# mills-lab/vapor

Measured on AMD Instinct MI355X. Metric: SV loci validated/sec, higher is better.
Workload: dtype u32

## Files before the change

### vapor_amd/build.py

```python
from __future__ import annotations

import hashlib
import os
import re
import subprocess
import sys

HERE = os.path.dirname(os.path.abspath(__file__))
ROOT = os.path.dirname(HERE)
SO = os.path.join(HERE, "libvapor_hip.so")
CSRC = os.path.join(HERE, "csrc")
SOURCES = [os.path.join(CSRC, "vapor_hip.hip"), os.path.join(CSRC, "vapor_bam.cpp")]
_HEADERS = [("vapor_kernels.h", True), ("vapor_wide.h", True), ("vapor_anyk.h", True), ("vapor_inflate.h", False),
            ("vapor_bamdev.h", True), ("vapor_fasta.h", True), ("vapor_refine.h", True), ("vapor_bgzf.h", False),
            ("vapor_records.h", True), ("vapor_planner.h", False), ("vapor_names.h", True),
            ("vapor_readrec.h", True), ("vapor_readplan.h", False), ("vapor_sa.h", False),
            ("vapor_realign.h", True), ("vapor_realign_plan.h", True),
            ("vapor_band_row.h", True),
            ("vapor_realign_trace.h", True), ("vapor_trace_plan.h", True),
            ("vapor_polish.h", True), ("vapor_polish_plan.h", True),
            ("vapor_junction.h", True), ("vapor_junction_plan.h", True),
            ("vapor_revote.h", True), ("vapor_revote_plan.h", True),
            ("vapor_polish_call.h", False),
            ("vapor_seqset_plan.h", False), ("vapor_image.h", False)]
DEPS = SOURCES + [os.path.join(CSRC, h) for h, _dev in _HEADERS] + [os.path.join(ROOT, "include", "vapor_hip.h")]
KERNEL_FILES = [os.path.join(CSRC, h) for h, dev in _HEADERS if dev] + [SOURCES[0], os.path.abspath(__file__)]

EXTRA_FLAGS = ["-mllvm", "-amdgpu-atomic-optimizer-strategy=None", "-mllvm", "-amdgpu-sched-strategy=max-ilp"]


def hipcc() -> str:
    for c in (os.environ.get("HIPCC"), "/opt/rocm/bin/hipcc", "hipcc"):
        if c and (os.path.isabs(c) and os.path.exists(c) or not os.path.isabs(c)):
            return c
    raise RuntimeError("hipcc not found")


_ID_RE = re.compile(rb"VAPOR_SOURCE_ID=([0-9a-f]{16}:[0-9a-f]{16})")

# ... 42 lines not shown
```

### vapor_amd/csrc/vapor_hip.hip

```cpp
#include "vapor_kernels.h"
#include "vapor_wide.h"
#include "vapor_anyk.h"
#include "vapor_realign.h"
#include "vapor_realign_trace.h"
#include "vapor_polish.h"
#include "vapor_revote.h"
#include "vapor_polish_call.h"
#include "vapor_seqset_plan.h"
#include "vapor_junction.h"
#include "vapor_bamdev.h"
#include "vapor_bgzf.h"
#include "vapor_fasta.h"
#include "vapor_refine.h"
#include "vapor_planner.h"
#include "vapor_readplan.h"
#include "vapor_hip.h"

#include <unistd.h>

#include <algorithm>
#include <cstdio>
#include <cstdlib>
#include <cstring>
#include <new>
#include <numeric>
#include <map>
#include <memory>
#include <mutex>
#include <set>
#include <string>
// ... 47 lines not shown
    bool user_stream = false;
    uint8_t* h_stage = nullptr;
    uint8_t* d_stage = nullptr;
    size_t stage_cap = 0;
    std::vector<double> h_gt;
    double* d_gt = nullptr;
    int reads_per_task = MAX_READS_PER_TASK;
    int n_cus = 256;
    int join_tasks = 256;
    int join_align = 1;
    int64_t max_pair_cap = (int64_t)1 << 28;
    bool shared_join = true;
    int remap_in_clean = 1;
    int clean_order = 1;
    int clean_fit = 1;
    int64_t trace_budget = vapor_trace::BUDGET_DEFAULT;
    int64_t anyk_edit_pairs = ANYK_EDIT_PAIRS;
    int stage_threads = 3;
    bool attrs_set = false;
    uint32_t* d_crc_pow = nullptr;
    std::map<const uint8_t*, size_t> arenas;
    hipStream_t bam_stream = nullptr;
    int bam_stream_share = 0;
    int bam_cu_share = 0;
    hipEvent_t bam_ev[2] = {nullptr, nullptr};
    double bam_stats[7] = {0, 0, 0, 0, 0, 0, 0};
    hipEvent_t fasta_ev[2] = {nullptr, nullptr};
    double fasta_stats[6] = {0, 0, 0, 0, 0, 0};
    BlockPool pool;
};
// ... 98 lines not shown
    vapor_ctx* ctx = nullptr;
    int device = 0;
    int32_t n = 0;
    int32_t n_lit = 0;
    std::vector<SeqDesc> h;
    SeqDesc* d_seqs = nullptr;
    uint32_t *d_p2 = nullptr, *d_e1 = nullptr, *d_x4 = nullptr;
    size_t plane_chunks = 0;
    std::vector<std::vector<HSeg>> derived;
    std::vector<ShareGroup> groups;
    std::vector<int32_t> group_of, slot_of;
    uint8_t* d_raw = nullptr;
    std::vector<int64_t> raw_off;
};

struct vapor_plan : PlanLayout {
    vapor_ctx* ctx = nullptr;
    int device = 0;
    vapor_seqset* set = nullptr;
    int64_t n_pairs = 0;
    std::vector<int64_t> last_stats;
    int hcap_want = 4096;
    bool hcap_measured = false;
    int64_t total_cap = 0;
    DPair* d_pairs = nullptr;
    DTask* d_tasks = nullptr;
    DTask* d_atasks = nullptr;
    int join_align = 0;
    PlanParams params{};
    bool aligned_made = false;
    int last_table = 0;
    int32_t* d_task_pairs = nullptr;
    unsigned long long* d_hits = nullptr;
    uint8_t* d_hflags = nullptr;
    unsigned long long* d_nhits = nullptr;
    long long* d_stats = nullptr;
    long long* h_stats = nullptr;
    hipEvent_t ev[4] = {nullptr, nullptr, nullptr, nullptr};
    hipEvent_t ev_f[2] = {nullptr, nullptr};
    std::vector<std::array<hipEvent_t, 4>> ring;
    int ring_n = 0;
    bool overflow_final = false;
    double acc_ms[4] = {0, 0, 0, 0};
    int64_t acc_n = 0;
    double* h_loci = nullptr;
    hipEvent_t ev_t0 = nullptr;
    hipStream_t lane = nullptr;
    int lane_ix = -1;
    hipStream_t fin = nullptr;
    hipEvent_t ev_clean = nullptr;
    hipEvent_t ev_fin = nullptr;
    bool have_fin = false;
    hipEvent_t ev_last = nullptr;
    hipEvent_t ev_after = nullptr;
    bool have_last = false, have_after = false;
    double t_join = 0, t_clean = 0, t_total = 0;
    int n_retried = 0;
    bool ran = false;
    bool flags_valid = false;
    int64_t n_reads = 0, n_loci = 0;
    DRead* d_reads = nullptr;
    int32_t* d_locus_first = nullptr;
    double* d_gt = nullptr;
    bool own_gt = false;
    double* d_read_scores = nullptr;
    double* d_loci = nullptr;
    unsigned int* d_overflow = nullptr;
    int32_t* d_big_list = nullptr;
    unsigned int* h_overflow = nullptr;
// ... 136 lines not shown
    if (!strcmp(name, "shared_join")) {
        c->shared_join = v != 0;
        return VAPOR_OK;
    }
    if (!strcmp(name, "remap_in_clean")) {
        if (v < 0 || v > 2) return fail(VAPOR_E_ARG, "vapor_set_param: remap_in_clean is 0, 1 or 2");
        c->remap_in_clean = (int)v;
        return VAPOR_OK;
    }
    if (!strcmp(name, "clean_order")) {
        c->clean_order = v != 0 ? 1 : 0;
        return VAPOR_OK;
    }
    if (!strcmp(name, "clean_fit")) {
        c->clean_fit = v != 0;
        return VAPOR_OK;
    }
    if (!strcmp(name, "trace_budget")) {
        c->trace_budget = vapor_trace::budget_of(v);
        return VAPOR_OK;
    }
    if (!strcmp(name, "anyk_edit_pairs")) {
        if (v < 1) return fail(VAPOR_E_ARG, "anyk_edit_pairs out of range");
        c->anyk_edit_pairs = v;
        return VAPOR_OK;
    }
    if (!strcmp(name, "stage_threads")) {
        if (v < 1 || v > 64) return fail(VAPOR_E_ARG, "stage_threads out of range");
        c->stage_threads = (int)v;
        return VAPOR_OK;
// ... 689 lines not shown
    dfree(p->ctx, p->d_hflags); p->d_hflags = nullptr;
    dfree(p->ctx, p->d_nhits); p->d_nhits = nullptr;
    dfree(p->ctx, p->d_stats); p->d_stats = nullptr;
    plan_free_reads(p);
    dfree(p->ctx, p->d_shares); p->d_shares = nullptr;
    dfree(p->ctx, p->d_maps); p->d_maps = nullptr;
    dfree(p->ctx, p->d_serve); p->d_serve = nullptr;
    dfree(p->ctx, p->d_clean_order); p->d_clean_order = nullptr;
    plan_free_grid(p);
}

extern "C" int vapor_plan_destroy(vapor_plan* p)
{
    if (!p) return VAPOR_OK;
    (void)hipSetDevice(p->device);
    if (p->ring_n > 0 && p->lane && ctx_alive(p->ctx)) {
        (void)hipStreamSynchronize(p->lane);
        if (p->fin) (void)hipStreamSynchronize(p->fin);
    }
    if (ctx_alive(p->ctx))
        for (auto& q : p->ctx->lane_plan)
            if (q == p) q = nullptr;
    plan_free_device(p);
    hfree(p->ctx, p->h_stats);
    hfree(p->ctx, p->h_overflow);
    dfree(p->ctx, p->d_overflow);
    dfree(p->ctx, p->d_big_list);
    for (auto& e : p->ev)
        if (e) (void)hipEventDestroy(e);
    for (auto& r : p->ring)
        for (auto& e : r)
            if (e) (void)hipEventDestroy(e);
    hfree(p->ctx, p->h_loci);
    for (auto& e : p->ev_f)
        if (e) (void)hipEventDestroy(e);
    if (p->ev_t0) (void)hipEventDestroy(p->ev_t0);
    if (p->ev_last) (void)hipEventDestroy(p->ev_last);
    if (p->ev_clean) (void)hipEventDestroy(p->ev_clean);
    if (p->ev_fin) (void)hipEventDestroy(p->ev_fin);
    if (p->ev_after) (void)hipEventDestroy(p->ev_after);
    delete p;
    return VAPOR_OK;
}

static_assert((2 * VAPOR_MAX_SEQ_LEN + 2 + 31) / 32 <= CLEAN_RANGE_WORDS_MAX, "cluster_axis sizes its per-thread word list for this");

static int plan_alloc_hits(vapor_plan* p)
{
    int64_t tot = 0;
    for (auto& d : p->hp) {
        d.hit_off = tot;
        tot += (int64_t)((d.cap + 3u) & ~3u);
    }
    tot += 4;
    HIPCHK(hipStreamSynchronize(p->ctx->stream));
    dfree(p->ctx, p->d_hits); p->d_hits = nullptr;
    dfree(p->ctx, p->d_hflags); p->d_hflags = nullptr;
    HIPCHK(dmalloc(p->ctx, (void**)&p->d_hits, (size_t)tot * sizeof(unsigned long long)));
    HIPCHK(dmalloc(p->ctx, (void**)&p->d_hflags, (size_t)tot));
    p->total_cap = tot;
// ... 17 lines not shown
    std::unique_ptr<vapor_plan, Building<vapor_plan, vapor_plan_destroy>> p(new (std::nothrow) vapor_plan(), {&sc});
    if (!p) return fail(VAPOR_E_NOMEM, "out of memory");
    p->ctx = ctx;
    p->device = ctx->device;
    p->set = set;
    p->n_pairs = n_pairs;
    p->params = PlanParams{ctx->reads_per_task, ctx->join_tasks, ctx->max_pair_cap, ctx->shared_join,
                           tile_pos<JoinCfg, 2>(), tile_pos<JoinCfg, 4>(), ctx->join_align == 2};
    static_cast<PlanLayout&>(*p) = plan_layout(p->params,
                                               SetView{set->h, set->n, set->n_lit, set->derived, set->groups, set->group_of, set->slot_of},
                                               n_pairs, pairs);
    p->join_align = ctx->join_align;
    if (p->join_align == 2) { p->tasks = p->atasks; p->launches = p->alaunches; p->model[0] = p->model[1]; }
    p->hcap_want = (int)std::min<int64_t>(p->hwant, CLEAN_HCAP_MAX);
    p->n_dpairs = (int64_t)p->shares.size();
    HIPCHK(dmalloc(ctx, (void**)&p->d_pairs, sizeof(DPair) * p->hp.size()));
    HIPCHK(dmalloc(ctx, (void**)&p->d_tasks, sizeof(DTask) * std::max<size_t>(p->tasks.size(), 1)));
    HIPCHK(dmalloc(ctx, (void**)&p->d_task_pairs, sizeof(int32_t) * std::max<size_t>(p->task_pairs.size(), 1)));
    HIPCHK(dmalloc(ctx, (void**)&p->d_nhits, sizeof(unsigned long long) * p->hp.size()));
    HIPCHK(hipMemsetAsync(p->d_nhits, 0, sizeof(unsigned long long) * p->hp.size(), ctx->stream));
    HIPCHK(dmalloc(ctx, (void**)&p->d_stats, sizeof(long long) * 16 * p->hp.size()));
    HIPCHK(hmalloc(ctx, (void**)&p->h_stats, sizeof(long long) * 16 * p->hp.size()));
    HIPCHK(dmalloc(ctx, (void**)&p->d_overflow, 4 * sizeof(unsigned int)));
    HIPCHK(hipMemsetAsync(p->d_overflow, 0, 4 * sizeof(unsigned int), ctx->stream));
    HIPCHK(dmalloc(ctx, (void**)&p->d_big_list, sizeof(int32_t) * p->hp.size()));
    HIPCHK(hmalloc(ctx, (void**)&p->h_overflow, 2 * sizeof(unsigned int)));
    if (p->n_dpairs) {
        HIPCHK(dmalloc(ctx, (void**)&p->d_shares, sizeof(DShare) * p->shares.size()));
        HIPCHK(dmalloc(ctx, (void**)&p->d_maps, sizeof(int32_t) * std::max<size_t>(p->tables.size(), 1)));
        HIPCHK(dmalloc(ctx, (void**)&p->d_serve, sizeof(DServe) * p->serve.size()));
// ... 58 lines not shown
}

static int clean_groups_lds(int rw, int hcap)
{
    const int g = std::min(clean_groups_cap(rw), std::max(hcap, 1));
    return 2 * std::max((g + 1) / 2, rw * 32 / 100 + 8);
}

static size_t clean_lds_bytes(int rw, int hcap, bool dual)
{
    const size_t bw = (size_t)rw + ((size_t)rw + 1) / 2;
    const size_t rec_word = ((dual ? 2 : 1) * bw + ((size_t)clean_groups_lds(rw, hcap) + 1) / 2 + 1) & ~(size_t)1;
    return sizeof(uint32_t) * rec_word + 64 + (size_t)hcap * 8 + 8;
}

struct CleanGeom { int hcap, per_cu; bool dual; };
static CleanGeom clean_geom_for(int range_words_cap, int want, bool dual, bool exact = false)
{
    CleanGeom g{0, 1, dual};
#ifdef VAPOR_DEV_BUILD
    if (const char* e = getenv("VAPOR_DEV_HCAP")) { g.hcap = atoi(e) & ~3; return g; }
#endif
    for (int per_cu = 2048 / CLEAN_THREADS; per_cu >= 1; --per_cu) {
        const size_t share = (size_t)(160 * 1024) / per_cu - 512;
        int cap = std::min(want, CLEAN_HCAP_MAX) & ~3;
        while (cap > 0 && clean_lds_bytes(range_words_cap, cap, dual) + 512 > share) cap -= 4;
        if (cap >= (exact ? want : want * 9 / 10) || per_cu == 1) { g.hcap = std::max(cap, 0); g.per_cu = per_cu; break; }
    }
    return g;
}
static CleanGeom clean_geom(int range_words_cap, int want, bool exact = false)
{
    const CleanGeom seq = clean_geom_for(range_words_cap, want, false, exact), dual = clean_geom_for(range_words_cap, want, true, exact);
#ifdef VAPOR_DEV_BUILD
    if (const char* e = getenv("VAPOR_DEV_CLEAN_DUAL")) return atoi(e) ? dual : seq;
#endif
    return dual.per_cu >= seq.per_cu ? dual : seq;
}

static int async_fold(vapor_plan* p);

static bool remap_in_clean(const vapor_plan* p)
{
    if (p->n_dpairs <= 0 || p->ctx->remap_in_clean == 0) return false;
    if (p->ctx->remap_in_clean == 2) return true;
    const CleanGeom cg = clean_geom(p->range_words_cap, p->hcap_want, p->hcap_measured);
    return p->n_pairs <= 4 * (int64_t)cg.per_cu * p->ctx->n_cus;
}

constexpr int JOIN_ALIGN_MIN_SAVING_PM = 15;
constexpr int JOIN_ALIGN_MAX_DEARER_PCT = 10;
static bool join_align_pays(const TableModel& bal, const TableModel& ali)
{
    return ali.n_tasks > 0 && (bal.sum - ali.sum) * 1000 >= bal.sum * JOIN_ALIGN_MIN_SAVING_PM && ali.path * 100 <= bal.path * (100 + JOIN_ALIGN_MAX_DEARER_PCT);
}
static int join_table_for_async(vapor_plan* p, hipStream_t st, int* table)
{
    *table = 0;
    if (p->join_align != 1) return VAPOR_OK;
    const vapor_ctx* c = p->ctx;
    if (c->user_stream || p->lane_ix < 0) return VAPOR_OK;
    const vapor_plan* o = c->lane_plan[1 - p->lane_ix];
    if (!o || o == p || o->ring_n <= 0) return VAPOR_OK;
    if (!p->aligned_made) {
        const vapor_seqset* s = p->set;
        plan_aligned(p->params, SetView{s->h, s->n, s->n_lit, s->derived, s->groups, s->group_of, s->slot_of}, p);
        p->aligned_made = true;
        if (!p->atasks.empty() && join_align_pays(p->model[0], p->model[1])) {
            HIPCHK(dmalloc(p->ctx, (void**)&p->d_atasks, sizeof(DTask) * p->atasks.size()));
            HIPCHK(hipMemcpyAsync(p->d_atasks, p->atasks.data(), sizeof(DTask) * p->atasks.size(), hipMemcpyHostToDevice, st));
        }
    }
    if (p->d_atasks) *table = 1;
    return VAPOR_OK;
}

static int plan_run_once(vapor_plan* p, int table, bool fetch_stats = true, hipEvent_t* evs = nullptr, hipStream_t on = nullptr, bool skip_big = false,
                         hipEvent_t before_clean = nullptr, bool keep_flags = true)
{
    vapor_ctx* c = p->ctx;
    hipStream_t st = on ? on : c->stream;
    hipEvent_t* ev = evs ? evs : p->ev;
    if (table == 1 && !p->d_atasks) table = 0;
    const std::vector<Launch>& launches = table == 1 ? p->alaunches : p->launches;
    const DTask* d_tasks = table == 1 ? p->d_atasks : p->d_tasks;
    p->last_table = table;
    if (launches.empty()) HIPCHK(hipMemsetAsync(p->d_overflow, 0, 2 * sizeof(unsigned int), st));
    HIPCHK(hipEventRecord(ev[0], st));
    bool first = true;
    for (const Launch& L : launches) {
        if (L.bps == 2) {
            if (L.k == 10) launch_join<2, 10>(p, L, d_tasks, first, st);
            else if (L.k == 20) launch_join<2, 20>(p, L, d_tasks, first, st);
            else if (L.k == 30) launch_join<2, 30>(p, L, d_tasks, first, st);
            else launch_join<2, 40>(p, L, d_tasks, first, st);
        } else {
            if (L.k == 10) launch_join<4, 10>(p, L, d_tasks, first, st);
            else if (L.k == 20) launch_join<4, 20>(p, L, d_tasks, first, st);
            else if (L.k == 30) launch_join<4, 30>(p, L, d_tasks, first, st);
            else launch_join<4, 40>(p, L, d_tasks, first, st);
        }
        first = false;
        HIPCHK(hipGetLastError());
    }
#if defined(VAPOR_AB) && VAPOR_AB == 3
    if (false) {
#else
    if (p->n_dpairs && !remap_in_clean(p)) {
#endif
        hipLaunchKernelGGL(remap_kernel, dim3((unsigned)p->n_dpairs), dim3(256), 0, st, (const DPair*)p->d_pairs, (const DShare*)p->d_shares,
                           (const int32_t*)p->d_maps, p->d_hits, p->d_nhits, p->d_overflow);
        HIPCHK(hipGetLastError());
    }
    HIPCHK(hipEventRecord(ev[1], st));
    if (before_clean) HIPCHK(hipStreamWaitEvent(st, before_clean, 0));
    if (p->n_pairs > 0) {
        const CleanGeom cg = clean_geom(p->range_words_cap, p->hcap_want, p->hcap_measured);
        const int hcap = cg.hcap;
        size_t lds = clean_lds_bytes(p->range_words_cap, hcap, cg.dual);
#ifdef VAPOR_DEV_BUILD
        if (const char* e = getenv("VAPOR_DEV_CLEAN_PAD")) lds += (size_t)atoi(e);
#endif
        const bool in_clean = remap_in_clean(p);
        launch_clean(p->range_words_cap, (unsigned)p->n_pairs, lds, st,
                     (const DPair*)p->d_pairs, (const int32_t*)p->d_clean_order, p->d_nhits,
                     p->d_hits, p->d_hflags, p->d_stats, p->range_words_cap,
                     clean_groups_lds(p->range_words_cap, hcap), hcap, p->d_overflow, p->d_big_list, skip_big ? 0 : 1, cg.dual ? 1 : 0,
                     in_clean ? (const DServe*)p->d_serve : (const DServe*)nullptr, (const int32_t*)p->d_maps, keep_flags ? 1 : 0);
        HIPCHK(hipGetLastError());
        p->flags_valid = keep_flags;
        if (!skip_big) {
            hipLaunchKernelGGL(clean_big_kernel, dim3((unsigned)std::min<int64_t>(p->n_pairs, CLEAN_BIG_GRID)), dim3(CLEAN_THREADS),
                               clean_fixed_bytes(p->range_words_cap, true), st, p->d_pairs, p->d_nhits, p->d_hits, p->d_hflags,
                               p->d_stats, p->range_words_cap, clean_groups_cap(p->range_words_cap), p->d_overflow, p->d_big_list);
            HIPCHK(hipGetLastError());
        }
    }
    HIPCHK(hipEventRecord(ev[2], st));
    if (p->n_pairs > 0 && fetch_stats)
        HIPCHK(hipMemcpyAsync(p->h_stats, p->d_stats, sizeof(long long) * 16 * (size_t)p->n_pairs, hipMemcpyDeviceToHost, st));
    if (!fetch_stats) return VAPOR_OK;
    HIPCHK(hipEventRecord(ev[3], st));
    HIPCHK(hipStreamSynchronize(st));
    float a = 0, b = 0, t = 0;
    HIPCHK(hipEventElapsedTime(&a, ev[0], ev[1]));
    HIPCHK(hipEventElapsedTime(&b, ev[1], ev[2]));
    HIPCHK(hipEventElapsedTime(&t, ev[0], ev[3]));
    p->t_join = a; p->t_clean = b; p->t_total = t;
    return VAPOR_OK;
}

extern "C" int vapor_plan_run(vapor_plan* p, int64_t* stats)
{
    if (!p || (p->n_pairs && !stats)) return fail(VAPOR_E_ARG, "vapor_plan_run: null argument");
    HIPCHK(hipSetDevice(p->ctx->device));
    if (p->ring_n > 0) {
        int rc0 = async_fold(p);
        if (rc0 != VAPOR_OK) return rc0;
    }
    p->n_retried = 0;
    for (int attempt = 0; attempt < 3; ++attempt) {
        int rc = plan_run_once(p, 0);
        if (rc != VAPOR_OK) return rc;
        int64_t grow = 0;
        for (int64_t i = 0; i < p->n_pairs; ++i) {
            const long long* s = p->h_stats + 16 * i;
            if (s[15] == VAPOR_E_OVERFLOW && s[14] <= p->ctx->max_pair_cap && (uint32_t)s[14] > p->hp[i].cap) {
                p->hp[i].cap = (uint32_t)s[14];
                ++grow;
            }
        }
// ... 8 lines not shown
        }
        if (!grow) break;
        p->n_retried += (int)grow;
        rc = plan_alloc_hits(p);
        if (rc != VAPOR_OK) return rc;
    }
    if (p->ctx->clean_fit && p->n_pairs > 0) {
        std::vector<unsigned long long> cnt((size_t)p->n_pairs);
        HIPCHK(hipMemcpy(cnt.data(), p->d_nhits, sizeof(unsigned long long) * cnt.size(), hipMemcpyDeviceToHost));
        uint32_t most = 0;
        for (int64_t i = 0; i < p->n_pairs; ++i)
            if (p->status[(size_t)i] == 0 && (uint32_t)(cnt[(size_t)i] >> 32) <= 65535u) most = std::max(most, (uint32_t)cnt[(size_t)i]);
        if (most > 0 && most <= (uint32_t)CLEAN_HCAP_MAX) {
            p->hcap_want = (int)((most + 3u) & ~3u);
            p->hcap_measured = true;
        }
    }
    if (p->n_dpairs) {
        std::vector<unsigned long long> dc((size_t)p->n_dpairs);
        HIPCHK(hipMemcpy(dc.data(), p->d_nhits + p->n_pairs, sizeof(unsigned long long) * dc.size(), hipMemcpyDeviceToHost));
        for (int64_t t = 0; t < p->n_dpairs; ++t)
            if ((uint32_t)dc[(size_t)t] > p->hp[(size_t)(p->n_pairs + t)].cap)
                for (int32_t tg : p->shares[(size_t)t].target)
                    if (tg >= 0 && p->status[(size_t)tg] == 0) p->status[(size_t)tg] = VAPOR_E_OVERFLOW;
    }
    for (int64_t i = 0; i < p->n_pairs; ++i) {
        long long* s = p->h_stats + 16 * i;
        if (p->status[i] != 0) {
            for (int t = 0; t < 16; ++t) s[t] = 0;
            s[1] = s[2] = -1;
            s[15] = p->status[i];
        }
    }
    memcpy(p->last_stats.data(), p->h_stats, sizeof(int64_t) * 16 * (size_t)p->n_pairs);
    memcpy(stats, p->h_stats, sizeof(int64_t) * 16 * (size_t)p->n_pairs);
    p->ran = true;
    return VAPOR_OK;
}

extern "C" int vapor_plan_timings(vapor_plan* p, double* ms, int32_t n)
{
    if (!p || !ms) return fail(VAPOR_E_ARG, "vapor_plan_timings: null argument");
    const CleanGeom cg = clean_geom(p->range_words_cap, p->hcap_want, p->hcap_measured);
    const TableModel& tm = p->model[p->last_table];
    double v[12] = {p->t_join, p->t_clean, p->t_total, (double)p->launches.size(), (double)p->n_retried, p->t_finish,
                    (double)p->n_served, (double)p->n_dpairs, (double)cg.per_cu, remap_in_clean(p) ? 1.0 : 0.0,
                    (double)tm.n_tasks, (double)tm.builds};
    for (int i = 0; i < n && i < 12; ++i) ms[i] = v[i];
    return VAPOR_OK;
}

extern "C" int vapor_plan_record_counts(vapor_plan* p, int64_t* records)
{
    if (!p || !records) return fail(VAPOR_E_ARG, "vapor_plan_record_counts: null argument");
    if (!p->ran) return fail(VAPOR_E_ARG, "vapor_plan_record_counts: plan has not been run");
    HIPCHK(hipSetDevice(p->ctx->device));
    std::vector<unsigned long long> cnt((size_t)std::max<int64_t>(p->n_pairs, 1));
    HIPCHK(hipMemcpy(cnt.data(), p->d_nhits, sizeof(unsigned long long) * (size_t)p->n_pairs, hipMemcpyDeviceToHost));
    for (int64_t i = 0; i < p->n_pairs; ++i) records[i] = (int64_t)(uint32_t)cnt[i];
    return VAPOR_OK;
}
// ... 9 lines not shown
        int64_t nh = p->ran ? p->last_stats[16 * i] : 0;
        b += (3 * n1 + 7) / 8 + (3 * n2 + 7) / 8 + 8 * nh + 128;
        c += n1 * n2;
    }
    *bytes = b;
    *cells = c;
    return VAPOR_OK;
}

extern "C" int vapor_plan_fetch_hits(vapor_plan* p, int64_t n_sel, const int64_t* pair_idx, int32_t* hits_ji,
                                     uint8_t* hit_flags, int64_t capacity, int64_t* hit_off)
{
    if (!p || n_sel < 0 || (n_sel && (!pair_idx || !hit_off))) return fail(VAPOR_E_ARG, "vapor_plan_fetch_hits: null argument");
    if (!p->ran) return fail(VAPOR_E_ARG, "vapor_plan_fetch_hits: plan has not been run");
    HIPCHK(hipSetDevice(p->ctx->device));
    if (hit_flags && (!p->flags_valid || p->ring_n > 0)) {
        int rc0 = vapor_plan_run(p, p->last_stats.data());
        if (rc0 != VAPOR_OK) return rc0;
    }
    std::vector<long long> off((size_t)n_sel + 1, 0), sel((size_t)std::max<int64_t>(n_sel, 1), 0);
    for (int64_t q = 0; q < n_sel; ++q) {
        int64_t i = pair_idx[q];
        if (i < 0 || i >= p->n_pairs) return fail(VAPOR_E_ARG, "pair index out of range");
        sel[q] = i;
        int64_t n = (p->last_stats[16 * i + 15] == 0) ? p->last_stats[16 * i] : 0;
        off[q + 1] = off[q] + n;
    }
    for (int64_t q = 0; q <= n_sel; ++q) hit_off[q] = off[q];
    if (off[n_sel] > capacity) return fail(VAPOR_E_OVERFLOW, "hit buffer too small");
    if (n_sel == 0 || off[n_sel] == 0) return VAPOR_OK;
    if (!hits_ji) return fail(VAPOR_E_ARG, "null hit buffer");
// ... 957 lines not shown
    HIPCHK(dmalloc(p->ctx, (void**)&p->d_grid, sizeof(int32_t) * block.size()));
    HIPCHK(dmalloc(p->ctx, (void**)&p->d_group_out, sizeof(double) * 16 * ng));
    HIPCHK(dmalloc(p->ctx, (void**)&p->d_winner_scores, sizeof(double) * (size_t)std::max<int32_t>(off[ng], 1)));
    HIPCHK(hipMemcpy(p->d_grid, block.data(), sizeof(int32_t) * block.size(), hipMemcpyHostToDevice));
    p->grid_score_off = off;
    p->n_grid_scores = off[ng];
    p->n_groups = n_groups;
    return VAPOR_OK;
}

extern "C" int vapor_plan_run_loci(vapor_plan* p, void* d_loci_out, double* loci_out, double* read_scores)
{
    if (!p) return fail(VAPOR_E_ARG, "vapor_plan_run_loci: null plan");
    if (!p->d_reads) return fail(VAPOR_E_ARG, "vapor_plan_run_loci: call vapor_plan_set_reads first");
    HIPCHK(hipSetDevice(p->ctx->device));
    if (p->ring_n > 0) {
        int rc0 = async_fold(p);
        if (rc0 != VAPOR_OK) return rc0;
    }
    hipStream_t st = p->ctx->stream;
    bool host_status = false;
    for (int64_t i = 0; i < p->n_pairs; ++i)
        if (p->status[i] != 0) { host_status = true; break; }
    int rc;
    const bool light = !(host_status || !p->ran);
    if (!light) {
        rc = vapor_plan_run(p, p->last_stats.data());
        if (rc != VAPOR_OK) return rc;
        for (int64_t i = 0; i < p->n_pairs && !host_status; ++i)
            if (p->status[i] != 0) host_status = true;
        if (host_status)
            HIPCHK(hipMemcpyAsync(p->d_stats, p->h_stats, sizeof(long long) * 16 * (size_t)p->n_pairs, hipMemcpyHostToDevice, st));
    } else {
        rc = plan_run_once(p, 0, false, nullptr, nullptr, false, nullptr, false);
        if (rc != VAPOR_OK) return rc;
    }
    hipEvent_t e1 = p->ev_f[1];
    double* d_out = d_loci_out ? static_cast<double*>(d_loci_out) : p->d_loci;
    if (p->n_loci > 0) {
        hipLaunchKernelGGL(finish_kernel, dim3((unsigned)p->n_loci), dim3(64), 0, st, p->d_reads, p->d_locus_first, p->d_stats,
                           p->d_gt, p->d_read_scores, d_out, (double*)nullptr);
        HIPCHK(hipGetLastError());
    }
    HIPCHK(hipEventRecord(e1, st));
    if (p->n_groups > 0 && p->n_loci > 0) {
// ... 158 lines not shown
            if (hipDeviceGetStreamPriorityRange(&lo, &hi) != hipSuccess ||
                hipStreamCreateWithPriority(&c->fin[l], hipStreamNonBlocking, hi) != hipSuccess) {
                (void)hipGetLastError();
                c->fin[l] = nullptr;
                HIPCHK(hipStreamCreateWithFlags(&c->fin[l], hipStreamNonBlocking));
            }
        }
        p->lane = c->lane[l];
        p->lane_ix = (int)l;
        p->fin = c->fin[l];
    }
    *out = p->lane;
    return VAPOR_OK;
}

static int async_fold(vapor_plan* p)
{
    hipStream_t st = nullptr;
    int rc = plan_lane(p, &st);
    if (rc != VAPOR_OK) return rc;
    if (p->lane && p->lane != st) HIPCHK(hipStreamSynchronize(p->lane));
    HIPCHK(hipStreamSynchronize(st));
    if (p->fin && p->fin != st) HIPCHK(hipStreamSynchronize(p->fin));
    for (int i = 0; i < p->ring_n; ++i) {
        float x = 0;
        hipEvent_t* ev = p->ring[(size_t)i].data();
        HIPCHK(hipEventElapsedTime(&x, ev[0], ev[1])); p->acc_ms[0] += x;
        HIPCHK(hipEventElapsedTime(&x, ev[1], ev[2])); p->acc_ms[1] += x;
        HIPCHK(hipEventElapsedTime(&x, ev[2], ev[3])); p->acc_ms[2] += x;
        HIPCHK(hipEventElapsedTime(&x, ev[0], ev[3])); p->acc_ms[3] += x;
    }
    p->acc_n += p->ring_n;
    p->ring_n = 0;
    return VAPOR_OK;
}

extern "C" int vapor_plan_run_loci_async(vapor_plan* p, void* d_loci_out)
{
    if (!p) return fail(VAPOR_E_ARG, "vapor_plan_run_loci_async: null plan");
    if (!p->d_reads) return fail(VAPOR_E_ARG, "vapor_plan_run_loci_async: call vapor_plan_set_reads first");
    if (!p->ran) return fail(VAPOR_E_ARG, "vapor_plan_run_loci_async: run the plan once with vapor_plan_run_loci first (it sizes the slots)");
    for (int64_t i = 0; i < p->n_pairs; ++i)
        if (p->status[i] != 0) return fail(VAPOR_E_ARG, "vapor_plan_run_loci_async: the plan holds pairs the host rejected; use vapor_plan_run_loci");
    HIPCHK(hipSetDevice(p->ctx->device));
    if (p->ring_n >= ASYNC_RING) {
        int rc0 = async_fold(p);
        if (rc0 != VAPOR_OK) return rc0;
    }
    hipStream_t st = nullptr;
    int rc = plan_lane(p, &st);
    if (rc != VAPOR_OK) return rc;
    if (p->ring.empty()) {
        p->ring.resize(ASYNC_RING);
        for (auto& r : p->ring)
            for (auto& e : r) { e = nullptr; HIPCHK(hipEventCreate(&e)); }
        HIPCHK(hmalloc(p->ctx, (void**)&p->h_loci, sizeof(double) * 8 * (size_t)std::max<int64_t>(p->n_loci, 1)));
        HIPCHK(hipEventCreateWithFlags(&p->ev_last, hipEventDisableTiming));
        HIPCHK(hipEventCreateWithFlags(&p->ev_clean, hipEventDisableTiming));
        HIPCHK(hipEventCreateWithFlags(&p->ev_fin, hipEventDisableTiming));
    }
    hipStream_t fs = (p->fin && !p->ctx->user_stream) ? p->fin : st;
    if (p->have_after) {
        HIPCHK(hipStreamWaitEvent(fs, p->ev_after, 0));
        p->have_after = false;
    }
    if (p->ring_n == 0 && p->acc_n == 0) HIPCHK(hipMemsetAsync(p->d_overflow + 2, 0, sizeof(unsigned int), st));
    hipEvent_t* ev = p->ring[(size_t)p->ring_n].data();
    int table = 0;
    rc = join_table_for_async(p, st, &table);
    if (rc != VAPOR_OK) return rc;
    rc = plan_run_once(p, table, false, ev, st, p->big_known && p->n_big == 0, (fs != st && p->have_fin) ? p->ev_fin : nullptr, false);
    if (rc != VAPOR_OK) return rc;
    double* d_out = d_loci_out ? static_cast<double*>(d_loci_out) : p->d_loci;
    if (fs != st) {
        HIPCHK(hipEventRecord(p->ev_clean, st));
        HIPCHK(hipStreamWaitEvent(fs, p->ev_clean, 0));
    }
    if (p->n_loci > 0) {
        hipLaunchKernelGGL(finish_kernel, dim3((unsigned)p->n_loci), dim3(64), 0, fs, p->d_reads, p->d_locus_first, p->d_stats,
                           p->d_gt, p->d_read_scores, d_out, p->h_loci);
        HIPCHK(hipGetLastError());
    }
    HIPCHK(hipEventRecord(ev[3], fs));
    HIPCHK(hipEventRecord(p->ev_last, fs));
    if (fs != st) {
        HIPCHK(hipEventRecord(p->ev_fin, fs));
        p->have_fin = true;
    }
    p->have_last = true;
    if (!p->ctx->user_stream && p->lane_ix >= 0) p->ctx->lane_plan[p->lane_ix] = p;
    ++p->ring_n;
    return VAPOR_OK;
}

extern "C" int vapor_plan_then(vapor_plan* p, void* hip_stream)
{
    if (!p) return fail(VAPOR_E_ARG, "vapor_plan_then: null plan");
    if (!p->have_last) return VAPOR_OK;
    HIPCHK(hipSetDevice(p->ctx->device));
    HIPCHK(hipStreamWaitEvent(static_cast<hipStream_t>(hip_stream), p->ev_last, 0));
    return VAPOR_OK;
}

extern "C" int vapor_plan_after(vapor_plan* p, void* hip_stream)
{
    if (!p) return fail(VAPOR_E_ARG, "vapor_plan_after: null plan");
    HIPCHK(hipSetDevice(p->ctx->device));
    if (!p->ev_after) HIPCHK(hipEventCreateWithFlags(&p->ev_after, hipEventDisableTiming));
    HIPCHK(hipEventRecord(p->ev_after, static_cast<hipStream_t>(hip_stream)));
    p->have_after = true;
    return VAPOR_OK;
}

extern "C" int vapor_plan_sync(vapor_plan* p, double* loci_out)
{
    if (!p) return fail(VAPOR_E_ARG, "vapor_plan_sync: null plan");
    HIPCHK(hipSetDevice(p->ctx->device));
    const int had = p->ring_n;
    int rc0 = async_fold(p);
    if (rc0 != VAPOR_OK) return rc0;
    if (p->acc_n > 0) {
        p->t_join = (float)(p->acc_ms[0] / p->acc_n); p->t_clean = (float)(p->acc_ms[1] / p->acc_n);
        p->t_finish = (float)(p->acc_ms[2] / p->acc_n); p->t_total = (float)(p->acc_ms[3] / p->acc_n);
        if (loci_out && p->n_loci && (had > 0 || p->h_loci)) memcpy(loci_out, p->h_loci, sizeof(double) * 8 * (size_t)p->n_loci);
    }
    p->acc_ms[0] = p->acc_ms[1] = p->acc_ms[2] = p->acc_ms[3] = 0;
    p->acc_n = 0;
    unsigned int sticky = 0;
    HIPCHK(hipMemcpy(&sticky, p->d_overflow + 2, sizeof(unsigned int), hipMemcpyDeviceToHost));
    if (sticky) {
        HIPCHK(hipMemset(p->d_overflow + 2, 0, sizeof(unsigned int)));
        return fail(VAPOR_E_OVERFLOW, "a pair outgrew its record slot during the asynchronous steps; run vapor_plan_run_loci (it resizes)" +
                    std::string(p->big_known ? "" : " [no blocking run has counted the pairs left to clean_big_kernel]") +
                    " [pairs left to clean_big_kernel on the last blocking run: " + std::to_string(p->n_big) + "]");
    }
    return VAPOR_OK;
}

#if defined(VAPOR_PHASE_TIMING) || defined(VAPOR_BLOCK_TIMING)
extern "C" int vapor_debug_block_ticks(double* out, int32_t n)
{
    std::vector<unsigned long long> h(4096);
// ... 39 lines not shown
```

Baseline: 817,700.

## Sample async timing events, cache clean geometry, and fold the event ring incrementally

Asynchronous runs now record timing events only on every Nth step (a new async_time_every setting, default 16). When the ring fills, they fold half of it by waiting on individual events instead of synchronizing whole streams. The clean geometry and remap-in-clean decision are computed once per plan rather than on every launch, and the host-status scan over all pairs is replaced with a cached flag. Timing events drop the system fence, and the separate finish event is merged into ev_last. The aim is to cut per-call host work and stream stalls on the enqueue path, at the cost of sampled rather than complete timing statistics.

```diff
diff --git a/vapor_amd/build.py b/vapor_amd/build.py
--- a/vapor_amd/build.py
+++ b/vapor_amd/build.py
@@ -22,7 +22,8 @@
             ("vapor_junction.h", True), ("vapor_junction_plan.h", True),
             ("vapor_revote.h", True), ("vapor_revote_plan.h", True),
             ("vapor_polish_call.h", False),
-            ("vapor_seqset_plan.h", False), ("vapor_image.h", False)]
+            ("vapor_seqset_plan.h", False), ("vapor_image.h", False),
+            ("vapor_async_ring.h", False)]
 DEPS = SOURCES + [os.path.join(CSRC, h) for h, _dev in _HEADERS] + [os.path.join(ROOT, "include", "vapor_hip.h")]
 KERNEL_FILES = [os.path.join(CSRC, h) for h, dev in _HEADERS if dev] + [SOURCES[0], os.path.abspath(__file__)]
 
diff --git a/vapor_amd/csrc/vapor_async_ring.h b/vapor_amd/csrc/vapor_async_ring.h
--- /dev/null
+++ b/vapor_amd/csrc/vapor_async_ring.h
@@ -0,0 +1,46 @@
+#pragma once
+
+#include <cstdint>
+
+namespace vapor {
+
+struct AsyncRing {
+    int size = 64;
+    int every = 16;
+    int head = 0;
+    int used = 0;
+    int64_t since = 0;
+    int64_t folded = 0;
+
+    struct Span { int first, n; };
+
+    int at(Span s, int i) const { return (s.first + i) % size; }
+
+    bool next_timed() const { return since % every == 0; }
+
+    Span must_fold() const { return used >= size ? Span{head, size / 2} : Span{head, 0}; }
+
+    Span in_use() const { return Span{head, used}; }
+
+    void fold(Span s)
+    {
+        head = (head + s.n) % size;
+        used -= s.n;
+        folded += s.n;
+        if (used == 0) head = 0;
+    }
+
+    int take()
+    {
+        if (used >= size) return -1;
+        return (head + used++) % size;
+    }
+
+    void enqueued() { ++since; }
+
+    void waited() { since = 0; }
+
+    void reported() { folded = 0; }
+};
+
+}
diff --git a/vapor_amd/csrc/vapor_hip.hip b/vapor_amd/csrc/vapor_hip.hip
--- a/vapor_amd/csrc/vapor_hip.hip
+++ b/vapor_amd/csrc/vapor_hip.hip
@@ -14,6 +14,7 @@
 #include "vapor_refine.h"
 #include "vapor_planner.h"
 #include "vapor_readplan.h"
+#include "vapor_async_ring.h"
 #include "vapor_hip.h"
 
 #include <unistd.h>
@@ -91,6 +92,7 @@
     int remap_in_clean = 1;
     int clean_order = 1;
     int clean_fit = 1;
+    int async_time_every = 16;
     int64_t trace_budget = vapor_trace::BUDGET_DEFAULT;
     int64_t anyk_edit_pairs = ANYK_EDIT_PAIRS;
     int stage_threads = 3;
@@ -219,6 +221,8 @@
     std::vector<int64_t> raw_off;
 };
 
+struct CleanGeom { int hcap, per_cu; bool dual; };
+
 struct vapor_plan : PlanLayout {
     vapor_ctx* ctx = nullptr;
     int device = 0;
@@ -227,6 +231,10 @@
     std::vector<int64_t> last_stats;
     int hcap_want = 4096;
     bool hcap_measured = false;
+    CleanGeom cg{0, 1, false};
+    bool cg_in_clean = false;
+    int cg_param = -1;
+    bool host_status = false;
     int64_t total_cap = 0;
     DPair* d_pairs = nullptr;
     DTask* d_tasks = nullptr;
@@ -244,20 +252,20 @@
     hipEvent_t ev[4] = {nullptr, nullptr, nullptr, nullptr};
     hipEvent_t ev_f[2] = {nullptr, nullptr};
     std::vector<std::array<hipEvent_t, 4>> ring;
-    int ring_n = 0;
+    AsyncRing ar;
     bool overflow_final = false;
     double acc_ms[4] = {0, 0, 0, 0};
-    int64_t acc_n = 0;
     double* h_loci = nullptr;
     hipEvent_t ev_t0 = nullptr;
     hipStream_t lane = nullptr;
     int lane_ix = -1;
     hipStream_t fin = nullptr;
     hipEvent_t ev_clean = nullptr;
-    hipEvent_t ev_fin = nullptr;
-    bool have_fin = false;
     hipEvent_t ev_last = nullptr;
     hipEvent_t ev_after = nullptr;
+#ifdef VAPOR_DEV_BUILD
+    hipEvent_t ev_dev_fin = nullptr;
+#endif
     bool have_last = false, have_after = false;
     double t_join = 0, t_clean = 0, t_total = 0;
     int n_retried = 0;
@@ -424,6 +432,11 @@
     }
     if (!strcmp(name, "clean_fit")) {
         c->clean_fit = v != 0;
+        return VAPOR_OK;
+    }
+    if (!strcmp(name, "async_time_every")) {
+        if (v < 1 || v > (1 << 20)) return fail(VAPOR_E_ARG, "async_time_every out of range (1 .. 2^20 steps a timed one)");
+        c->async_time_every = (int)v;
         return VAPOR_OK;
     }
     if (!strcmp(name, "trace_budget")) {
@@ -1143,7 +1156,7 @@
 {
     if (!p) return VAPOR_OK;
     (void)hipSetDevice(p->device);
-    if (p->ring_n > 0 && p->lane && ctx_alive(p->ctx)) {
+    if (p->ar.since > 0 && p->lane && ctx_alive(p->ctx)) {
         (void)hipStreamSynchronize(p->lane);
         if (p->fin) (void)hipStreamSynchronize(p->fin);
     }
@@ -1166,13 +1179,17 @@
     if (p->ev_t0) (void)hipEventDestroy(p->ev_t0);
     if (p->ev_last) (void)hipEventDestroy(p->ev_last);
     if (p->ev_clean) (void)hipEventDestroy(p->ev_clean);
-    if (p->ev_fin) (void)hipEventDestroy(p->ev_fin);
+#ifdef VAPOR_DEV_BUILD
+    if (p->ev_dev_fin) (void)hipEventDestroy(p->ev_dev_fin);
+#endif
     if (p->ev_after) (void)hipEventDestroy(p->ev_after);
     delete p;
     return VAPOR_OK;
 }
 
 static_assert((2 * VAPOR_MAX_SEQ_LEN + 2 + 31) / 32 <= CLEAN_RANGE_WORDS_MAX, "cluster_axis sizes its per-thread word list for this");
+
+static void plan_geom_make(vapor_plan* p);
 
 static int plan_alloc_hits(vapor_plan* p)
 {
@@ -1220,6 +1237,8 @@
     if (p->join_align == 2) { p->tasks = p->atasks; p->launches = p->alaunches; p->model[0] = p->model[1]; }
     p->hcap_want = (int)std::min<int64_t>(p->hwant, CLEAN_HCAP_MAX);
     p->n_dpairs = (int64_t)p->shares.size();
+    plan_geom_make(p.get());
+    p->host_status = std::any_of(p->status.begin(), p->status.end(), [](int32_t x) { return x != 0; });
     HIPCHK(dmalloc(ctx, (void**)&p->d_pairs, sizeof(DPair) * p->hp.size()));
     HIPCHK(dmalloc(ctx, (void**)&p->d_tasks, sizeof(DTask) * std::max<size_t>(p->tasks.size(), 1)));
     HIPCHK(dmalloc(ctx, (void**)&p->d_task_pairs, sizeof(int32_t) * std::max<size_t>(p->task_pairs.size(), 1)));
@@ -1308,7 +1327,6 @@
     return sizeof(uint32_t) * rec_word + 64 + (size_t)hcap * 8 + 8;
 }
 
-struct CleanGeom { int hcap, per_cu; bool dual; };
 static CleanGeom clean_geom_for(int range_words_cap, int want, bool dual, bool exact = false)
 {
     CleanGeom g{0, 1, dual};
@@ -1334,12 +1352,22 @@
 
 static int async_fold(vapor_plan* p);
 
-static bool remap_in_clean(const vapor_plan* p)
+static bool remap_in_clean(const vapor_plan* p, const CleanGeom& cg)
 {
     if (p->n_dpairs <= 0 || p->ctx->remap_in_clean == 0) return false;
     if (p->ctx->remap_in_clean == 2) return true;
-    const CleanGeom cg = clean_geom(p->range_words_cap, p->hcap_want, p->hcap_measured);
     return p->n_pairs <= 4 * (int64_t)cg.per_cu * p->ctx->n_cus;
+}
+
+static void plan_geom_make(vapor_plan* p)
+{
+    p->cg = clean_geom(p->range_words_cap, p->hcap_want, p->hcap_measured);
+    p->cg_in_clean = remap_in_clean(p, p->cg);
+    p->cg_param = p->ctx->remap_in_clean;
+}
+static inline void plan_geom(vapor_plan* p)
+{
+    if (p->cg_param != p->ctx->remap_in_clean) plan_geom_make(p);
 }
 
 constexpr int JOIN_ALIGN_MIN_SAVING_PM = 15;
@@ -1355,7 +1383,7 @@
     const vapor_ctx* c = p->ctx;
     if (c->user_stream || p->lane_ix < 0) return VAPOR_OK;
     const vapor_plan* o = c->lane_plan[1 - p->lane_ix];
-    if (!o || o == p || o->ring_n <= 0) return VAPOR_OK;
+    if (!o || o == p || o->ar.since <= 0) return VAPOR_OK;
     if (!p->aligned_made) {
         const vapor_seqset* s = p->set;
         plan_aligned(p->params, SetView{s->h, s->n, s->n_lit, s->derived, s->groups, s->group_of, s->slot_of}, p);
@@ -1370,7 +1398,7 @@
 }
 
 static int plan_run_once(vapor_plan* p, int table, bool fetch_stats = true, hipEvent_t* evs = nullptr, hipStream_t on = nullptr, bool skip_big = false,
-                         hipEvent_t before_clean = nullptr, bool keep_flags = true)
+                         hipEvent_t before_clean = nullptr, bool keep_flags = true, bool timed = true)
 {
     vapor_ctx* c = p->ctx;
     hipStream_t st = on ? on : c->stream;
@@ -1380,7 +1408,8 @@
     const DTask* d_tasks = table == 1 ? p->d_atasks : p->d_tasks;
     p->last_table = table;
     if (launches.empty()) HIPCHK(hipMemsetAsync(p->d_overflow, 0, 2 * sizeof(unsigned int), st));
-    HIPCHK(hipEventRecord(ev[0], st));
+    plan_geom(p);
+    if (timed) HIPCHK(hipEventRecord(ev[0], st));
     bool first = true;
     for (const Launch& L : launches) {
         if (L.bps == 2) {
@@ -1400,22 +1429,22 @@
 #if defined(VAPOR_AB) && VAPOR_AB == 3
     if (false) {
 #else
-    if (p->n_dpairs && !remap_in_clean(p)) {
+    if (p->n_dpairs && !p->cg_in_clean) {
 #endif
         hipLaunchKernelGGL(remap_kernel, dim3((unsigned)p->n_dpairs), dim3(256), 0, st, (const DPair*)p->d_pairs, (const DShare*)p->d_shares,
                            (const int32_t*)p->d_maps, p->d_hits, p->d_nhits, p->d_overflow);
         HIPCHK(hipGetLastError());
     }
-    HIPCHK(hipEventRecord(ev[1], st));
+    if (timed) HIPCHK(hipEventRecord(ev[1], st));
     if (before_clean) HIPCHK(hipStreamWaitEvent(st, before_clean, 0));
     if (p->n_pairs > 0) {
-        const CleanGeom cg = clean_geom(p->range_words_cap, p->hcap_want, p->hcap_measured);
+        const CleanGeom& cg = p->cg;
         const int hcap = cg.hcap;
         size_t lds = clean_lds_bytes(p->range_words_cap, hcap, cg.dual);
 #ifdef VAPOR_DEV_BUILD
         if (const char* e = getenv("VAPOR_DEV_CLEAN_PAD")) lds += (size_t)atoi(e);
 #endif
-        const bool in_clean = remap_in_clean(p);
+        const bool in_clean = p->cg_in_clean;
         launch_clean(p->range_words_cap, (unsigned)p->n_pairs, lds, st,
                      (const DPair*)p->d_pairs, (const int32_t*)p->d_clean_order, p->d_nhits,
                      p->d_hits, p->d_hflags, p->d_stats, p->range_words_cap,
@@ -1430,7 +1459,7 @@
             HIPCHK(hipGetLastError());
         }
     }
-    HIPCHK(hipEventRecord(ev[2], st));
+    if (timed) HIPCHK(hipEventRecord(ev[2], st));
     if (p->n_pairs > 0 && fetch_stats)
         HIPCHK(hipMemcpyAsync(p->h_stats, p->d_stats, sizeof(long long) * 16 * (size_t)p->n_pairs, hipMemcpyDeviceToHost, st));
     if (!fetch_stats) return VAPOR_OK;
@@ -1448,7 +1477,7 @@
 {
     if (!p || (p->n_pairs && !stats)) return fail(VAPOR_E_ARG, "vapor_plan_run: null argument");
     HIPCHK(hipSetDevice(p->ctx->device));
-    if (p->ring_n > 0) {
+    if (p->ar.since > 0) {
         int rc0 = async_fold(p);
         if (rc0 != VAPOR_OK) return rc0;
     }
@@ -1487,6 +1516,7 @@
         if (most > 0 && most <= (uint32_t)CLEAN_HCAP_MAX) {
             p->hcap_want = (int)((most + 3u) & ~3u);
             p->hcap_measured = true;
+            plan_geom_make(p);
         }
     }
     if (p->n_dpairs) {
@@ -1495,7 +1525,7 @@
         for (int64_t t = 0; t < p->n_dpairs; ++t)
             if ((uint32_t)dc[(size_t)t] > p->hp[(size_t)(p->n_pairs + t)].cap)
                 for (int32_t tg : p->shares[(size_t)t].target)
-                    if (tg >= 0 && p->status[(size_t)tg] == 0) p->status[(size_t)tg] = VAPOR_E_OVERFLOW;
+                    if (tg >= 0 && p->status[(size_t)tg] == 0) { p->status[(size_t)tg] = VAPOR_E_OVERFLOW; p->host_status = true; }
     }
     for (int64_t i = 0; i < p->n_pairs; ++i) {
         long long* s = p->h_stats + 16 * i;
@@ -1514,10 +1544,11 @@
 extern "C" int vapor_plan_timings(vapor_plan* p, double* ms, int32_t n)
 {
     if (!p || !ms) return fail(VAPOR_E_ARG, "vapor_plan_timings: null argument");
-    const CleanGeom cg = clean_geom(p->range_words_cap, p->hcap_want, p->hcap_measured);
+    plan_geom(p);
+    const CleanGeom& cg = p->cg;
     const TableModel& tm = p->model[p->last_table];
     double v[12] = {p->t_join, p->t_clean, p->t_total, (double)p->launches.size(), (double)p->n_retried, p->t_finish,
-                    (double)p->n_served, (double)p->n_dpairs, (double)cg.per_cu, remap_in_clean(p) ? 1.0 : 0.0,
+                    (double)p->n_served, (double)p->n_dpairs, (double)cg.per_cu, p->cg_in_clean ? 1.0 : 0.0,
                     (double)tm.n_tasks, (double)tm.builds};
     for (int i = 0; i < n && i < 12; ++i) ms[i] = v[i];
     return VAPOR_OK;
@@ -1557,7 +1588,7 @@
     if (!p || n_sel < 0 || (n_sel && (!pair_idx || !hit_off))) return fail(VAPOR_E_ARG, "vapor_plan_fetch_hits: null argument");
     if (!p->ran) return fail(VAPOR_E_ARG, "vapor_plan_fetch_hits: plan has not been run");
     HIPCHK(hipSetDevice(p->ctx->device));
-    if (hit_flags && (!p->flags_valid || p->ring_n > 0)) {
+    if (hit_flags && (!p->flags_valid || p->ar.since > 0)) {
         int rc0 = vapor_plan_run(p, p->last_stats.data());
         if (rc0 != VAPOR_OK) return rc0;
     }
@@ -2545,21 +2576,18 @@
     if (!p) return fail(VAPOR_E_ARG, "vapor_plan_run_loci: null plan");
     if (!p->d_reads) return fail(VAPOR_E_ARG, "vapor_plan_run_loci: call vapor_plan_set_reads first");
     HIPCHK(hipSetDevice(p->ctx->device));
-    if (p->ring_n > 0) {
+    if (p->ar.since > 0) {
         int rc0 = async_fold(p);
         if (rc0 != VAPOR_OK) return rc0;
     }
     hipStream_t st = p->ctx->stream;
-    bool host_status = false;
-    for (int64_t i = 0; i < p->n_pairs; ++i)
-        if (p->status[i] != 0) { host_status = true; break; }
+    bool host_status = p->host_status;
     int rc;
     const bool light = !(host_status || !p->ran);
     if (!light) {
         rc = vapor_plan_run(p, p->last_stats.data());
         if (rc != VAPOR_OK) return rc;
-        for (int64_t i = 0; i < p->n_pairs && !host_status; ++i)
-            if (p->status[i] != 0) host_status = true;
+        host_status = p->host_status;
         if (host_status)
             HIPCHK(hipMemcpyAsync(p->d_stats, p->h_stats, sizeof(long long) * 16 * (size_t)p->n_pairs, hipMemcpyHostToDevice, st));
     } else {
@@ -2748,6 +2776,30 @@
     return VAPOR_OK;
 }
 
+#ifdef VAPOR_DEV_BUILD
+static bool dev_on(const char* name) { const char* e = getenv(name); return e && atoi(e) != 0; }
+static const bool DEV_ASYNC_FENCE = dev_on("VAPOR_DEV_ASYNC_FENCE");
+static const bool DEV_ASYNC_TWO_FIN = dev_on("VAPOR_DEV_ASYNC_TWO_FIN");
+static const bool DEV_ASYNC_DRAIN = dev_on("VAPOR_DEV_ASYNC_DRAIN");
+static const bool DEV_ASYNC_CLEAN_NOFENCE = dev_on("VAPOR_DEV_ASYNC_CLEAN_NOFENCE");
+#else
+constexpr bool DEV_ASYNC_FENCE = false, DEV_ASYNC_DRAIN = false, DEV_ASYNC_CLEAN_NOFENCE = false;
+#endif
+
+static int async_fold_sets(vapor_plan* p, AsyncRing::Span s)
+{
+    for (int i = 0; i < s.n; ++i) {
+        float x = 0;
+        hipEvent_t* ev = p->ring[(size_t)p->ar.at(s, i)].data();
+        HIPCHK(hipEventElapsedTime(&x, ev[0], ev[1])); p->acc_ms[0] += x;
+        HIPCHK(hipEventElapsedTime(&x, ev[1], ev[2])); p->acc_ms[1] += x;
+        HIPCHK(hipEventElapsedTime(&x, ev[2], ev[3])); p->acc_ms[2] += x;
+        HIPCHK(hipEventElapsedTime(&x, ev[0], ev[3])); p->acc_ms[3] += x;
+    }
+    p->ar.fold(s);
+    return VAPOR_OK;
+}
+
 static int async_fold(vapor_plan* p)
 {
     hipStream_t st = nullptr;
@@ -2756,17 +2808,9 @@
     if (p->lane && p->lane != st) HIPCHK(hipStreamSynchronize(p->lane));
     HIPCHK(hipStreamSynchronize(st));
     if (p->fin && p->fin != st) HIPCHK(hipStreamSynchronize(p->fin));
-    for (int i = 0; i < p->ring_n; ++i) {
-        float x = 0;
-        hipEvent_t* ev = p->ring[(size_t)i].data();
-        HIPCHK(hipEventElapsedTime(&x, ev[0], ev[1])); p->acc_ms[0] += x;
-        HIPCHK(hipEventElapsedTime(&x, ev[1], ev[2])); p->acc_ms[1] += x;
-        HIPCHK(hipEventElapsedTime(&x, ev[2], ev[3])); p->acc_ms[2] += x;
-        HIPCHK(hipEventElapsedTime(&x, ev[0], ev[3])); p->acc_ms[3] += x;
-    }
-    p->acc_n += p->ring_n;
-    p->ring_n = 0;
-    return VAPOR_OK;
+    rc = async_fold_sets(p, p->ar.in_use());
+    p->ar.waited();
+    return rc;
 }
 
 extern "C" int vapor_plan_run_loci_async(vapor_plan* p, void* d_loci_out)
@@ -2774,36 +2818,48 @@
     if (!p) return fail(VAPOR_E_ARG, "vapor_plan_run_loci_async: null plan");
     if (!p->d_reads) return fail(VAPOR_E_ARG, "vapor_plan_run_loci_async: call vapor_plan_set_reads first");
     if (!p->ran) return fail(VAPOR_E_ARG, "vapor_plan_run_loci_async: run the plan once with vapor_plan_run_loci first (it sizes the slots)");
-    for (int64_t i = 0; i < p->n_pairs; ++i)
-        if (p->status[i] != 0) return fail(VAPOR_E_ARG, "vapor_plan_run_loci_async: the plan holds pairs the host rejected; use vapor_plan_run_loci");
+    if (p->host_status) return fail(VAPOR_E_ARG, "vapor_plan_run_loci_async: the plan holds pairs the host rejected; use vapor_plan_run_loci");
     HIPCHK(hipSetDevice(p->ctx->device));
-    if (p->ring_n >= ASYNC_RING) {
-        int rc0 = async_fold(p);
-        if (rc0 != VAPOR_OK) return rc0;
-    }
     hipStream_t st = nullptr;
     int rc = plan_lane(p, &st);
     if (rc != VAPOR_OK) return rc;
     if (p->ring.empty()) {
         p->ring.resize(ASYNC_RING);
+        p->ar.size = ASYNC_RING;
         for (auto& r : p->ring)
-            for (auto& e : r) { e = nullptr; HIPCHK(hipEventCreate(&e)); }
+            for (auto& e : r) { e = nullptr; HIPCHK(hipEventCreateWithFlags(&e, DEV_ASYNC_FENCE ? hipEventDefault : hipEventDisableSystemFence)); }
         HIPCHK(hmalloc(p->ctx, (void**)&p->h_loci, sizeof(double) * 8 * (size_t)std::max<int64_t>(p->n_loci, 1)));
         HIPCHK(hipEventCreateWithFlags(&p->ev_last, hipEventDisableTiming));
-        HIPCHK(hipEventCreateWithFlags(&p->ev_clean, hipEventDisableTiming));
-        HIPCHK(hipEventCreateWithFlags(&p->ev_fin, hipEventDisableTiming));
+        HIPCHK(hipEventCreateWithFlags(&p->ev_clean, hipEventDisableTiming | (DEV_ASYNC_CLEAN_NOFENCE ? hipEventDisableSystemFence : 0)));
+#ifdef VAPOR_DEV_BUILD
+        if (DEV_ASYNC_TWO_FIN) HIPCHK(hipEventCreateWithFlags(&p->ev_dev_fin, hipEventDisableTiming));
+#endif
+    }
+    if (p->ar.since == 0) p->ar.every = p->ctx->async_time_every;
+    const bool timed = p->ar.next_timed();
+    if (timed) {
+        const AsyncRing::Span half = p->ar.must_fold();
+        if (half.n > 0) {
+            if (DEV_ASYNC_DRAIN) {
+                HIPCHK(hipStreamSynchronize(st));
+                if (p->fin && p->fin != st) HIPCHK(hipStreamSynchronize(p->fin));
+            }
+            for (int i = half.n - 1; i >= 0; --i) HIPCHK(hipEventSynchronize(p->ring[(size_t)p->ar.at(half, i)][3]));
+            int rc0 = async_fold_sets(p, half);
+            if (rc0 != VAPOR_OK) return rc0;
+        }
     }
     hipStream_t fs = (p->fin && !p->ctx->user_stream) ? p->fin : st;
     if (p->have_after) {
         HIPCHK(hipStreamWaitEvent(fs, p->ev_after, 0));
         p->have_after = false;
     }
-    if (p->ring_n == 0 && p->acc_n == 0) HIPCHK(hipMemsetAsync(p->d_overflow + 2, 0, sizeof(unsigned int), st));
-    hipEvent_t* ev = p->ring[(size_t)p->ring_n].data();
+    if (p->ar.since == 0 && p->ar.folded == 0) HIPCHK(hipMemsetAsync(p->d_overflow + 2, 0, sizeof(unsigned int), st));
+    hipEvent_t* ev = timed ? p->ring[(size_t)p->ar.take()].data() : nullptr;
     int table = 0;
     rc = join_table_for_async(p, st, &table);
     if (rc != VAPOR_OK) return rc;
-    rc = plan_run_once(p, table, false, ev, st, p->big_known && p->n_big == 0, (fs != st && p->have_fin) ? p->ev_fin : nullptr, false);
+    rc = plan_run_once(p, table, false, ev, st, p->big_known && p->n_big == 0, (fs != st && p->have_last) ? p->ev_last : nullptr, false, timed);
     if (rc != VAPOR_OK) return rc;
     double* d_out = d_loci_out ? static_cast<double*>(d_loci_out) : p->d_loci;
     if (fs != st) {
@@ -2815,15 +2871,14 @@
                            p->d_gt, p->d_read_scores, d_out, p->h_loci);
         HIPCHK(hipGetLastError());
     }
-    HIPCHK(hipEventRecord(ev[3], fs));
+    if (timed) HIPCHK(hipEventRecord(ev[3], fs));
     HIPCHK(hipEventRecord(p->ev_last, fs));
-    if (fs != st) {
-        HIPCHK(hipEventRecord(p->ev_fin, fs));
-        p->have_fin = true;
-    }
+#ifdef VAPOR_DEV_BUILD
+    if (DEV_ASYNC_TWO_FIN && fs != st) HIPCHK(hipEventRecord(p->ev_dev_fin, fs));
+#endif
     p->have_last = true;
     if (!p->ctx->user_stream && p->lane_ix >= 0) p->ctx->lane_plan[p->lane_ix] = p;
-    ++p->ring_n;
+    p->ar.enqueued();
     return VAPOR_OK;
 }
 
@@ -2850,16 +2905,17 @@
 {
     if (!p) return fail(VAPOR_E_ARG, "vapor_plan_sync: null plan");
     HIPCHK(hipSetDevice(p->ctx->device));
-    const int had = p->ring_n;
+    const bool had = p->ar.since > 0;
     int rc0 = async_fold(p);
     if (rc0 != VAPOR_OK) return rc0;
-    if (p->acc_n > 0) {
-        p->t_join = (float)(p->acc_ms[0] / p->acc_n); p->t_clean = (float)(p->acc_ms[1] / p->acc_n);
-        p->t_finish = (float)(p->acc_ms[2] / p->acc_n); p->t_total = (float)(p->acc_ms[3] / p->acc_n);
-        if (loci_out && p->n_loci && (had > 0 || p->h_loci)) memcpy(loci_out, p->h_loci, sizeof(double) * 8 * (size_t)p->n_loci);
+    if (p->ar.folded > 0) {
+        const double n = (double)p->ar.folded;
+        p->t_join = (float)(p->acc_ms[0] / n); p->t_clean = (float)(p->acc_ms[1] / n);
+        p->t_finish = (float)(p->acc_ms[2] / n); p->t_total = (float)(p->acc_ms[3] / n);
+        if (loci_out && p->n_loci && (had || p->h_loci)) memcpy(loci_out, p->h_loci, sizeof(double) * 8 * (size_t)p->n_loci);
     }
     p->acc_ms[0] = p->acc_ms[1] = p->acc_ms[2] = p->acc_ms[3] = 0;
-    p->acc_n = 0;
+    p->ar.reported();
     unsigned int sticky = 0;
     HIPCHK(hipMemcpy(&sticky, p->d_overflow + 2, sizeof(unsigned int), hipMemcpyDeviceToHost));
     if (sticky) {
```

Result: no change. 825,300 (median of 6 runs) (+0.9%).
